# VealFang/PLI-SLAM

Hardware: AMD Instinct MI355X
Metric: stereo frames/sec (ORB+LSD extract+match), 752x480 EuRoC (higher is better)
Workload: dtype u8; 1 GPU; 1xMI355X: 752x480 stereo pairs, extract + stereo Hamming match (BASELINE configs[1] shape, batched); 752x480, 1200 ORB kp (8 levels x1.2) + LSD/LBD (<=100 lines); 256 stereo frames per GPU per step; frames_per_gpu=256, parallelism=frame-batch data parallel, 1 rank(s), gather of result tables to rank 0

## Files before the change

### pli_slam_amd/csrc/lsd_rect.hpp

```cpp
#pragma once
#include "kernels.hpp"
#include "device_prims.hpp"

namespace pli {

constexpr double RX_PI = 3.14159265358979323846;
constexpr double RX_DEG2RAD = RX_PI / 180;
constexpr double RX_3_2_PI = (3 * RX_PI) / 2;
constexpr double RX_2PI = 2 * RX_PI;

__device__ __forceinline__ double rx_angle_diff(double a, double b) {
  double diff = a - b;
  while (diff <= -RX_PI) diff += RX_2PI;
  while (diff > RX_PI) diff -= RX_2PI;
  return fabs(diff);
}

constexpr int RX_RECT_GROUP_MAX = 192;
constexpr int RX_RECT_CACHE = 4;

template <int LANES>
__device__ __forceinline__ void rx_rect_region(bool on, const RxRect& it, const DevParams& P, const float4* __restrict__ rec,
                                               const double* __restrict__ mg, const int* __restrict__ arena,
                                               float4* __restrict__ rgSeg, double (*st)[64], double (*wc)[64], int (*ec)[64], int rmask,
                                               const int2* __restrict__ hot = nullptr ,
                                               const float2* __restrict__ cold = nullptr ) {
  const int lane = threadIdx.x & 63, gl = lane & (LANES - 1), g0 = lane & ~(LANES - 1);
  const int W = P.LW;
  const double prec = P.prec;
  const int cnt = on ? it.cnt : 0;
  const int* lst = arena + it.off;
  const double reg_angle = (double)fast_atan2_deg(it.sumdy, it.sumdx) * RX_DEG2RAD;
  int cmax = cnt;
#pragma unroll
  for (int o = 32; o >= LANES; o >>= 1) cmax = max(cmax, __shfl_xor(cmax, o, 64));
  double acc = 0.0;
  for (int c0 = 0; c0 < cmax; c0 += LANES) {
    const int kk = c0 + gl;
    double v0 = 0.0, v1 = 0.0, v2 = 0.0;
    if (kk < cnt) {
      const int e = lst[kk];
      const int ex = e & 0xFFFF, ey = e >> 16;
      const double w = mg ? mg[ey * W + ex] : sqrt((double)__float_as_int(rec[ey * W + ex].w) / 4.0);
      v0 = (double)ex * w;
      v1 = (double)ey * w;
      v2 = w;
      if (c0 < RX_RECT_CACHE * LANES) { wc[c0 / LANES][lane] = w; ec[c0 / LANES][lane] = e; }
    }
    wave_lds_sync();
    st[0][lane] = v0; st[1][lane] = v1; st[2][lane] = v2;
    wave_lds_sync();
    if (gl < 3 && c0 < cnt) {
      const int mm = (min(LANES, cnt - c0) + 7) & ~7;
      for (int tt = 0; tt < mm; tt += 8) {
        double a[8];
#pragma unroll
        for (int u = 0; u < 8; ++u) a[u] = st[gl][g0 + tt + u];
#pragma unroll
        for (int u = 0; u < 8; ++u) acc += a[u];
      }
    }
  }
  const double cq = acc / __shfl(acc, g0 + 2, 64);
  const double x = __shfl(cq, g0, 64), y = __shfl(cq, g0 + 1, 64);
  acc = 0.0;
  for (int c0 = 0; c0 < cmax; c0 += LANES) {
    const int kk = c0 + gl;
    double v0 = 0.0, v1 = 0.0, v2 = 0.0;
    if (kk < cnt) {
      const bool cached = c0 < RX_RECT_CACHE * LANES;
      const int e = cached ? ec[c0 / LANES][lane] : lst[kk];
      const int ex = e & 0xFFFF, ey = e >> 16;
      const double w = cached ? wc[c0 / LANES][lane] : (mg ? mg[ey * W + ex] : sqrt((double)__float_as_int(rec[ey * W + ex].w) / 4.0));
      const double dx = (double)ex - x, dy = (double)ey - y;
      v0 = dy * dy * w;
      v1 = dx * dx * w;
      v2 = dx * dy * w;
    }
    wave_lds_sync();
    st[0][lane] = v0; st[1][lane] = v1; st[2][lane] = v2;
    wave_lds_sync();
    if (gl < 3 && c0 < cnt) {
      const int mm = (min(LANES, cnt - c0) + 7) & ~7;
      for (int tt = 0; tt < mm; tt += 8) {
        double a[8];
#pragma unroll
        for (int u = 0; u < 8; ++u) a[u] = st[gl][g0 + tt + u];
        if (gl < 2) {
#pragma unroll
          for (int u = 0; u < 8; ++u) acc += a[u];
        } else {
#pragma unroll
          for (int u = 0; u < 8; ++u) acc -= a[u];
        }
      }
    }
  }
  const double Ixx = __shfl(acc, g0, 64), Iyy = __shfl(acc, g0 + 1, 64), Ixy = __shfl(acc, g0 + 2, 64);
  const double lambda = 0.5 * (Ixx + Iyy - sqrt((Ixx - Iyy) * (Ixx - Iyy) + 4.0 * Ixy * Ixy));
  const bool wide = fabs(Ixx) > fabs(Iyy);
  double theta = (double)fast_atan2_deg(wide ? (float)(lambda - Ixx) : (float)Ixy, wide ? (float)Ixy : (float)(lambda - Iyy));
  theta *= RX_DEG2RAD;
  double adiff = rx_angle_diff(theta, reg_angle);
  {
    const bool need = on && it.approx != 0 && hot != nullptr && fabs(adiff - prec) < P.rectApproxBand;
    if (__builtin_amdgcn_ballot_w64(need)) {
      int cm = need ? cnt : 0;
#pragma unroll
      for (int o = 32; o >= LANES; o >>= 1) cm = max(cm, __shfl_xor(cm, o, 64));
      float sx = 0.f, sy = 0.f;
      for (int c0 = 0; c0 < cm; c0 += LANES) {
        const int kk = c0 + gl;
        float cy = 0.f, cz = 0.f;
        if (need && kk < cnt) {
          const int e = lst[kk];
          const int p = (e >> 16) * W + (e & 0xFFFF);
          if (kk == 0) {
            double sn, cs;
            sincos((double)__int_as_float(hot[p].x) * RX_DEG2RAD, &sn, &cs);
            cy = (float)cs; cz = (float)sn;
          } else if (cold) {
            const float2 cp = cold[p];
            cy = cp.x; cz = cp.y;
          } else {
            const float4 r = rec[p];
            cy = r.y; cz = r.z;
          }
        }
        for (int j = 0; j < LANES; ++j) {
          const float vy = __shfl(cy, g0 + j, 64), vz = __shfl(cz, g0 + j, 64);
          if (need && c0 + j < cnt) {
            sx = (c0 + j == 0) ? vy : __fadd_rn(sx, vy);
            sy = (c0 + j == 0) ? vz : __fadd_rn(sy, vz);
          }
        }
      }
      if (need) adiff = rx_angle_diff(theta, (double)fast_atan2_deg(sy, sx) * RX_DEG2RAD);
    }
  }
  if (adiff > prec) theta += RX_PI;
  double dxr, dyr;
  sincos(theta, &dyr, &dxr);
  double l_min = 0, l_max = 0;
  for (int kk = gl; kk < cnt; kk += LANES) {
    const int e = kk < RX_RECT_CACHE * LANES ? ec[kk / LANES][lane] : lst[kk];
    const double l = ((double)(e & 0xFFFF) - x) * dxr + ((double)(e >> 16) - y) * dyr;
    l_max = fmax(l_max, l);
    l_min = fmin(l_min, l);
  }
#pragma unroll
  for (int o = LANES / 2; o > 0; o >>= 1) {
    l_max = fmax(l_max, __shfl_xor(l_max, o, 64));
    l_min = fmin(l_min, __shfl_xor(l_min, o, 64));
  }
  double e = ((gl & 1) ? y : x) + ((gl & 2) ? l_max : l_min) * ((gl & 1) ? dyr : dxr);
  e += 0.5;
  const double scale = P.lsdScale;
  if (scale != 1) e /= scale;
  if (on && gl < 4) reinterpret_cast<float*>(&rgSeg[it.rank & rmask])[gl] = (float)e;
}


__device__ __forceinline__ void rx_rect_wave(const DevParams& P, const RxCtl& c, const float4* __restrict__ rec, const double* __restrict__ mg,
                                             const int* __restrict__ arena, const RxRect* __restrict__ rects, int rectCap,
                                             float4* __restrict__ rgSeg, int first, int stride, double (*st)[64], double (*wc)[64],
                                             int (*ec)[64], int rmask = -1, const int2* __restrict__ hot = nullptr,
                                             const float2* __restrict__ cold = nullptr) {
  const int nrect = min((int)(c.rectArena >> RX_ARENA_BITS), rectCap);
  const int lane = threadIdx.x & 63, g = lane >> 4;
  for (int w0 = first * 4; w0 < nrect; w0 += stride * 4) {
    RxRect it = {0, 0, 0, 1.f, 0.f, 0};
    const bool have = w0 + g < nrect;
    if (have) it = rects[w0 + g];
    const bool small = have && it.cnt <= RX_RECT_GROUP_MAX;
    if (__builtin_amdgcn_ballot_w64(small)) rx_rect_region<16>(small, it, P, rec, mg, arena, rgSeg, st, wc, ec, rmask, hot, cold);
    unsigned long long big = __builtin_amdgcn_ballot_w64(have && !small) & 0x0001000100010001ull;
    while (big) {
      const int gl0 = __ffsll((long long)big) - 1;
      big &= big - 1ull;
      RxRect bt;
      bt.rank = __shfl(it.rank, gl0, 64); bt.off = __shfl(it.off, gl0, 64); bt.cnt = __shfl(it.cnt, gl0, 64);
      bt.sumdx = __shfl(it.sumdx, gl0, 64); bt.sumdy = __shfl(it.sumdy, gl0, 64); bt.approx = __shfl(it.approx, gl0, 64);
      rx_rect_region<64>(true, bt, P, rec, mg, arena, rgSeg, st, wc, ec, rmask, hot, cold);
    }
  }
}

}
```

### pli_slam_amd/csrc/lsd_relax.hip

```cpp
#include "kernels.hpp"
#include "device_prims.hpp"
#include "lsd_rect.hpp"
#include <climits>
#include <type_traits>

namespace pli {

constexpr float RX_NOTDEF = -1024.f;
constexpr int RX_INF = LSD_ID_INF;

__device__ __forceinline__ int2 rx_load_own(const int2* p) {
  unsigned long long v = __hip_atomic_load(reinterpret_cast<const unsigned long long*>(p), __ATOMIC_RELAXED,
                                           __HIP_MEMORY_SCOPE_AGENT);
  return make_int2((int)(v & 0xFFFFFFFFull), (int)(v >> 32));
}

__device__ __forceinline__ int rx_lds_read(const int* p) {
  typedef __attribute__((address_space(3))) const volatile int lds_cvint;
  return *(lds_cvint*)p;
}


__device__ __forceinline__ int rx_block_append(bool flag, int* counter, int* lds) {
  const int tid = threadIdx.x, lane = tid & 63, wv = tid >> 6, nw = blockDim.x >> 6;
// ... 542 lines not shown
          cnt = 1; k = 0;
          bx0 = bx1 = sd.xy & 0xFFFF; by0 = by1 = sd.xy >> 16;
        } else {
          const RxHand& hd = hand[wi - nbig];
          r = hd.rank; cnt = hd.cnt; k = hd.k;
          sumdx = hd.sumdx; sumdy = hd.sumdy;
          reg_angle = (double)fast_atan2_deg(sumdy, sumdx) * RX_DEG2RAD;
          bx0 = hd.box0 & 0xFFFF; by0 = hd.box0 >> 16; bx1 = hd.box1 & 0xFFFF; by1 = hd.box1 >> 16;
          for (int i = gl; i < cnt; i += RX_GL) q[i] = hd.q[i];
        }
        r = U(r); cnt = U(cnt); k = U(k);
        bx0 = U(bx0); bx1 = U(bx1); by0 = U(by0); by1 = U(by1);
        sumdx = Uf(sumdx); sumdy = Uf(sumdy);
      }
    }
    if constexpr (RX_GL == 64) { active = U(active) != 0; exhausted = U(exhausted) != 0; }
    if (!__builtin_amdgcn_ballot_w64(active)) break;
    __builtin_amdgcn_fence(__ATOMIC_RELEASE, "wavefront");
    bool dead = false, accepted = false;
    int qi = 0, nb = 0;
    raced = raced || pendOld <= r;
    asm volatile("" ::"v"(pendOld) : "memory");
    pendOld = 0x7FFFFFFF;
    auto step = [&](auto spillTag) {
      constexpr bool SPILL = decltype(spillTag)::value;
      int myxy = -1;
      qi = -1;
      float4 rr = make_float4(RX_NOTDEF, 0.f, 0.f, 0.f);
      int2 oo = make_int2(0, 0);
      nb = active ? min(NP, cnt - k) : 0;
      if (pi < nb) {
        const int e = SPILL ? qget(k + pi) : rx_lds_read(&q[k + pi]);
        const int nx = (e & 0xFFFF) + ndx, ny = (e >> 16) + ndy;
        if (nx >= 0 && ny >= 0 && nx < W && ny < H) {
          qi = ny * W + nx;
          myxy = (ny << 16) | nx;
          rr = rec[qi];
          oo = rx_load_own(&own[qi]);
        }
      }
      const int prevv = ci ? oo.x : oo.y, curv = ci ? oo.y : oo.x;
      const bool cand = rr.x != RX_NOTDEF && !(prevv < r || curv <= r);
      const double ad = (double)rr.x * RX_DEG2RAD;
      unsigned long long rem = (__builtin_amdgcn_ballot_w64(cand) >> gbase) & GMASK;
      dead = false; accepted = false;
      while (__builtin_amdgcn_ballot_w64(rem != 0)) {
        double n_theta = fabs(reg_angle - ad);
        if (n_theta > RX_3_2_PI) {
          n_theta = fabs(n_theta - RX_2PI);
        }
        const unsigned long long m = ((__builtin_amdgcn_ballot_w64(cand && n_theta <= prec) >> gbase) & GMASK) & rem;
        if (!m) { rem = 0; continue; }
        const int j2 = __ffsll((long long)m) - 1;
        rem &= ~((2ull << j2) - 1ull);
        const float cj = bcast(rr.y, j2), sj = bcast(rr.z, j2);
        const int xyj = __float_as_int(bcast(__int_as_float(myxy), j2));
        const int qj = __float_as_int(bcast(__int_as_float(qi), j2));
        rem &= ~((__builtin_amdgcn_ballot_w64(qi == qj) >> gbase) & GMASK);
        const int ax = xyj & 0xFFFF, ay = xyj >> 16;
        accepted = accepted || gl == j2;
        if (!SPILL || cnt < RX_GQ) {
          q[cnt] = xyj;
        } else {
          const int o = cnt - RX_GQ;
          if (o % RX_BBLK == 0) {
            int nbk = 0;
            if (o / RX_BBLK >= RX_BMAXBLK) { dead = true; rem = 0; continue; }
            if (gl == 0) {
              const unsigned long long ra = atomicAdd(&c.rectArena, (unsigned long long)RX_BBLK) & ((1ull << RX_ARENA_BITS) - 1ull);
              nbk = ra + RX_BBLK > (unsigned long long)arenaCap ? -1 : (int)ra;
            }
            nbk = __shfl(nbk, gbase, 64);
            if (nbk < 0) { dead = true; rem = 0; continue; }
            gb[o / RX_BBLK] = nbk;
          }
          if (gl == 0) arena[gb[o / RX_BBLK] + o % RX_BBLK] = xyj;
          __threadfence_block();
        }
        ++cnt;
        bx0 = min(bx0, ax); bx1 = max(bx1, ax); by0 = min(by0, ay); by1 = max(by1, ay);
        sumdx = __fadd_rn(sumdx, cj);
        sumdy = __fadd_rn(sumdy, sj);
        reg_angle = (double)fast_atan2_deg(sumdy, sumdx) * RX_DEG2RAD;
      }
    };
    if (__builtin_amdgcn_ballot_w64(active && cnt + 8 * NP + 1 > RX_GQ)) step(std::true_type{});
    else step(std::false_type{});
    if (accepted) pendOld = __hip_atomic_fetch_min(ci ? &own[qi].y : &own[qi].x, r, __ATOMIC_RELAXED, __HIP_MEMORY_SCOPE_AGENT);
    if (active) {
      k += nb;
      if (dead) { c.overflow = 5; active = false; exhausted = true; }
      else if (k >= cnt) {
        active = false;
        if (raced || pendOld <= r) atomicAdd(&c.races, 1);
        raced = false; pendOld = 0x7FFFFFFF;
        if (gl == 0) {
          rgSize[r] = cnt;
          rgBox[r] = make_int2((by0 << 16) | bx0, (by1 << 16) | bx1);
        }
        if (cnt >= minReg) {
          int off = 0, slot = 0;
          if (gl == 0) {
            const unsigned long long ra = atomicAdd(&c.rectArena, (1ull << RX_ARENA_BITS) | (unsigned long long)cnt);
            const unsigned long long o64 = ra & ((1ull << RX_ARENA_BITS) - 1ull);
            off = o64 + cnt > (unsigned long long)arenaCap ? -1 : (int)o64;
            slot = (int)(ra >> RX_ARENA_BITS);
          }
          off = __shfl(off, gbase, 64); slot = __shfl(slot, gbase, 64);
          if (off < 0 || slot >= rectCap) c.overflow = off < 0 ? 3 : 4;
          else {
            for (int i = gl; i < cnt; i += RX_GL) arena[off + i] = qget(i);
            if (gl == 0) {
              RxRect& it = rects[slot];
              it.rank = r; it.off = off; it.cnt = cnt; it.sumdx = sumdx; it.sumdy = sumdy; it.approx = 0;
            }
          }
        }
      }
    }
  }
}

__global__ __launch_bounds__(64) void k_rx_grow_big(const DevParams* __restrict__ Pp, RxCtl* __restrict__ ctl,
                                                    const float4* __restrict__ recAll, int2* __restrict__ ownAll,
                                                    const RxSeed* __restrict__ bigAll, int bigCap,
                                                    const RxHand* __restrict__ handAll, int handCap,
                                                    int* __restrict__ rgSizeAll, int2* __restrict__ rgBoxAll,
                                                    int* __restrict__ arenaAll, int arenaCap,
                                                    RxRect* __restrict__ rectAll, int rectCap, int img0, int t) {
  rx_grow_groups<32, 512>(Pp, ctl, recAll, ownAll, bigAll, bigCap, handAll, handCap, rgSizeAll, rgBoxAll, arenaAll, arenaCap,
                          rectAll, rectCap, img0, t);
}

__global__ __launch_bounds__(64) void k_rx_grow_wave(const DevParams* __restrict__ Pp, RxCtl* __restrict__ ctl,
                                                     const float4* __restrict__ recAll, int2* __restrict__ ownAll,
                                                     const RxSeed* __restrict__ bigAll, int bigCap,
                                                     const RxHand* __restrict__ handAll, int handCap,
                                                     int* __restrict__ rgSizeAll, int2* __restrict__ rgBoxAll,
                                                     int* __restrict__ arenaAll, int arenaCap,
                                                     RxRect* __restrict__ rectAll, int rectCap, int img0, int t) {
  rx_grow_groups<64, 1024>(Pp, ctl, recAll, ownAll, bigAll, bigCap, handAll, handCap, rgSizeAll, rgBoxAll, arenaAll, arenaCap,
                           rectAll, rectCap, img0, t);
}

#endif

__global__ __launch_bounds__(64) void k_rx_rect(const DevParams* __restrict__ Pp, RxCtl* __restrict__ ctl,
                                                const float4* __restrict__ recAll, const int* __restrict__ arenaAll,
                                                int arenaCap, const RxRect* __restrict__ rectAll, int rectCap,
                                                float4* __restrict__ rgSegAll, int img0, const double* __restrict__ mgAll, int rmask,
                                                const int2* __restrict__ hotAll ,
                                                const float2* __restrict__ coldAll ) {
  __shared__ double st[3][64];
  __shared__ double wc[RX_RECT_CACHE][64];
  __shared__ int ec[RX_RECT_CACHE][64];
  const DevParams& P = *Pp;
  const int img = blockIdx.y + img0;
  const RxCtl& c = ctl[img];
  if (c.state == 2 || c.overflow) return;
  const int64_t npix = (int64_t)P.LW * P.LH;
  rx_rect_wave(P, c, recAll + img * npix, mgAll ? mgAll + img * npix : nullptr ,
               arenaAll + (int64_t)img * arenaCap, rectAll + (int64_t)img * rectCap, rectCap, rgSegAll + img * npix, blockIdx.x, gridDim.x, st, wc, ec, rmask,
               hotAll ? hotAll + img * npix : nullptr, coldAll ? coldAll + img * npix : nullptr);
}

constexpr int RX_CCHUNK = 2048;

__device__ __forceinline__ bool rx_emits(const int* order, const int2* own, int size, int i, int n, int minReg, const int2* box, int boxCut) {
  if (i >= n) return false;
  if (size < minReg || own[order[i]].x != i) return false;
  if (boxCut < 0) return true;
  const int2 b = box[i];
  return lsd_box_can_pass(b.x, b.y, boxCut);
}

__global__ __launch_bounds__(256) void k_rx_count(const RxCtl* __restrict__ ctl, const int* __restrict__ orderAll,
                                                  const int* __restrict__ nDefined, const int2* __restrict__ ownAll,
                                                  const int* __restrict__ rgSizeAll, int* __restrict__ chunkCntAll,
                                                  int nChunks, int64_t npix, int minReg, int img0, const int2* __restrict__ rgBoxAll,
                                                  int boxCut) {
  __shared__ int wsum[4];
  const int img = blockIdx.y + img0;
  if (ctl[img].state != 2 || ctl[img].overflow) return;
  const int n = nDefined[img];
  const int tid = threadIdx.x;
  int cntv = 0;
  int sz[RX_CCHUNK / 256];
#pragma unroll
  for (int j = 0; j < RX_CCHUNK / 256; ++j) sz[j] = rgSizeAll[img * npix + min((int)blockIdx.x * RX_CCHUNK + j * 256 + tid, max(n - 1, 0))];
#pragma unroll
  for (int j = 0; j < RX_CCHUNK / 256; ++j)
    cntv += rx_emits(orderAll + img * npix, ownAll + img * npix, sz[j], blockIdx.x * RX_CCHUNK + j * 256 + tid, n, minReg,
                     rgBoxAll + img * npix, boxCut) ? 1 : 0;
  cntv = wave_sum_i32(cntv);
  if ((tid & 63) == 0) wsum[tid >> 6] = cntv;
  __syncthreads();
  if (tid == 0) chunkCntAll[(int64_t)img * nChunks + blockIdx.x] = wsum[0] + wsum[1] + wsum[2] + wsum[3];
}

__global__ __launch_bounds__(256) void k_rx_emit(const RxCtl* __restrict__ ctl, const int* __restrict__ orderAll,
                                                 const int* __restrict__ nDefined, const int2* __restrict__ ownAll,
                                                 const int* __restrict__ rgSizeAll, const float4* __restrict__ rgSegAll,
                                                 const int* __restrict__ chunkCntAll, int nChunks, int64_t npix,
                                                 int minReg, float* __restrict__ segAll, int* __restrict__ nSeg,
                                                 int maxSeg, int img0, const int2* __restrict__ rgBoxAll, int boxCut) {
  __shared__ int wsum[4];
  __shared__ int sbase;
  const int img = blockIdx.y + img0;
  if (ctl[img].state != 2 || ctl[img].overflow) return;
  const int n = nDefined[img];
  const int tid = threadIdx.x, lane = tid & 63, wv = tid >> 6;
  const int* cc = chunkCntAll + (int64_t)img * nChunks;
  int part = 0;
  for (int j = tid; j < (int)blockIdx.x; j += 256) part += cc[j];
  part = wave_sum_i32(part);
  if (lane == 0) wsum[wv] = part;
  __syncthreads();
  if (tid == 0) sbase = wsum[0] + wsum[1] + wsum[2] + wsum[3];
  __syncthreads();
  int base = sbase;
  float* seg = segAll + (int64_t)img * maxSeg * 4;
  int sz[RX_CCHUNK / 256];
#pragma unroll
  for (int j = 0; j < RX_CCHUNK / 256; ++j) sz[j] = rgSizeAll[img * npix + min((int)blockIdx.x * RX_CCHUNK + j * 256 + tid, max(n - 1, 0))];
#pragma unroll
  for (int j = 0; j < RX_CCHUNK / 256; ++j) {
    const int i = blockIdx.x * RX_CCHUNK + j * 256 + tid;
    const bool e = rx_emits(orderAll + img * npix, ownAll + img * npix, sz[j], i, n, minReg, rgBoxAll + img * npix, boxCut);
    const unsigned long long bal = __builtin_amdgcn_ballot_w64(e);
    __syncthreads();
    if (lane == 0) wsum[wv] = __popcll(bal);
    __syncthreads();
    int pos = base + __popcll(bal & ((1ull << lane) - 1ull));
    for (int w2 = 0; w2 < wv; ++w2) pos += wsum[w2];
    if (e && pos < maxSeg) {
      const float4 v = rgSegAll[img * npix + i];
      seg[4 * pos + 0] = v.x; seg[4 * pos + 1] = v.y; seg[4 * pos + 2] = v.z; seg[4 * pos + 3] = v.w;
    }
    base += wsum[0] + wsum[1] + wsum[2] + wsum[3];
  }
  if ((int)blockIdx.x == nChunks - 1 && tid == 0) nSeg[img] = min(base, maxSeg);
}

}
```

### pli_slam_amd/csrc/lsd_tile.hip

```cpp
#include "kernels.hpp"
#include "device_prims.hpp"
#include "lsd_rect.hpp"
#include <climits>
#include <type_traits>

namespace pli {

constexpr float TX_NOTDEF = -1024.f;
constexpr int TX_INF = LSD_ID_INF;
constexpr double TX_PI = 3.14159265358979323846;
constexpr double TX_DEG2RAD = TX_PI / 180;
constexpr double TX_3_2_PI = (3 * TX_PI) / 2;
constexpr double TX_2PI = 2 * TX_PI;
#if !defined(PLI_DEV) && (defined(TX_CLAIM_SCOPE) || defined(TX_GROUP) || defined(TX_OWN_LOAD) || defined(TX_DIAG_PAD) || defined(TX_DIAG_NOWAIT) || defined(TX_DIAG_HOT_NOFOLD))
#error "diagnostic builds of lsd_tile.hip need -DPLI_DEV"
#endif
#ifndef TX_CLAIM_SCOPE
#define TX_CLAIM_SCOPE __HIP_MEMORY_SCOPE_AGENT
#endif
#ifndef TX_GROUP
#define TX_GROUP 8
#endif
static_assert(TX_GROUP == 0 || TX_GROUP == 2 || TX_GROUP == 4 || TX_GROUP == 8, "a group member is an octet of lanes");
constexpr int TX_GQ = 768;
// ... 1776 lines not shown
}
#ifdef PLI_DEV
__global__ __launch_bounds__(64) __attribute__((amdgpu_waves_per_eu(8, 8))) void k_tx_grow_spec(TxRound A, int t) {
  __shared__ int q[TX_GQ_SPEC];
  __shared__ int gb[TX_BMAXBLK];
  __shared__ int park[8 * 64];
  tx_grow_tile<false, true, TX_GQ_SPEC>(A, blockIdx.y + A.img0, blockIdx.x, t, q, gb, park);
}
#endif
__global__ __launch_bounds__(64) __attribute__((amdgpu_waves_per_eu(8, 8))) void k_tx_grow_sparse(TxRound A, int t) {
  __shared__ int q[TX_GQ];
  __shared__ int gb[TX_BMAXBLK];
  __shared__ int park[TX_PARK];
  tx_grow_tile<true>(A, blockIdx.y + A.img0, blockIdx.x, t, q, gb, park);
}
__global__ __launch_bounds__(64) __attribute__((amdgpu_waves_per_eu(8, 8))) void k_tx_grow_sparse_h(TxRound A, int t) {
  __shared__ int q[TX_GQ];
  __shared__ int gb[TX_BMAXBLK + 4];
  __shared__ int park[TX_PARK];
  tx_grow_tile<true, false, TX_GQ, 0, true>(A, blockIdx.y + A.img0, blockIdx.x, t, q, gb, park);
}

__global__ __launch_bounds__(256) void k_tx_rec_from_hot(const RxCtl* __restrict__ ctl, const int2* __restrict__ hotAll,
                                                         const float2* __restrict__ coldAll, float4* __restrict__ recAll, int64_t npix, int img0) {
  const int img = blockIdx.y + img0;
  if (ctl[img].state == 2 && ctl[img].overflow == 0) return;
  for (int64_t p = (int64_t)blockIdx.x * 256 + threadIdx.x; p < npix; p += (int64_t)gridDim.x * 256) {
    const float2 cp = coldAll[img * npix + p];
    recAll[img * npix + p] = make_float4(__int_as_float(hotAll[img * npix + p].x), cp.x == TX_NOTDEF ? 0.f : cp.x, cp.y, 0.f);
  }
}


__global__ __launch_bounds__(256) void k_tx_collect(RxCtl* __restrict__ ctl, const int* __restrict__ idPlaneAll, const int2* __restrict__ ownAll,
                                                    const int* __restrict__ rgSizeAll, int64_t npix, int minReg, int* __restrict__ candAll,
                                                    int* __restrict__ candCnt, int img0, int emitCap, const int2* __restrict__ rgBoxAll,
                                                    int boxCut) {
  constexpr int CAP = 1024;
  __shared__ int s_n, s_base;
  __shared__ int s_buf[CAP];
  const int img = blockIdx.y + img0;
  RxCtl& c = ctl[img];
  if (c.state != 2 || c.overflow) return;
  const int64_t base = (int64_t)img * npix;
  const int tid = threadIdx.x, lane = tid & 63;
  int* cand = candAll + (int64_t)img * TX_EMIT_CAP;
  if (tid == 0) s_n = 0;
  __syncthreads();
  const int* rgSize = rgSizeAll + base;
  const bool vec = (npix & 3) == 0 && ((uintptr_t)rgSize & 15) == 0;
  for (int64_t p1 = (int64_t)blockIdx.x * 4096; p1 < npix; p1 += (int64_t)gridDim.x * 4096) {
    int sz[16];
#pragma unroll
    for (int u = 0; u < 4; ++u) {
      const int64_t p = p1 + u * 1024 + tid * 4;
      int4 v = make_int4(0, 0, 0, 0);
      if (vec && p + 3 < npix) v = *reinterpret_cast<const int4*>(rgSize + p);
      else {
        if (p < npix) v.x = rgSize[p];
        if (p + 1 < npix) v.y = rgSize[p + 1];
        if (p + 2 < npix) v.z = rgSize[p + 2];
        if (p + 3 < npix) v.w = rgSize[p + 3];
      }
      sz[4 * u] = v.x; sz[4 * u + 1] = v.y; sz[4 * u + 2] = v.z; sz[4 * u + 3] = v.w;
    }
    unsigned hits = 0u;
#pragma unroll
    for (int j = 0; j < 16; ++j) hits |= (sz[j] >= minReg ? 1u : 0u) << j;
    while (hits) {
      const int j = __ffs(hits) - 1;
      hits &= hits - 1u;
      const int64_t p = p1 + (j >> 2) * 1024 + tid * 4 + (j & 3);
      const int id = idPlaneAll[base + p];
      const int2 box = boxCut >= 0 ? rgBoxAll[base + p] : make_int2(0, 0);
      if (id == TX_INF || ownAll[base + p].x != id || !lsd_box_can_pass(box.x, box.y, boxCut)) continue;
      const int at = atomicAdd(&s_n, 1);
      if (at < CAP) s_buf[at] = id;
      else {
        const int g = atomicAdd(&candCnt[img], 1);
        if (g < emitCap) cand[g] = id;
        else c.overflow = 6;
      }
    }
  }
  __syncthreads();
  const int n = min(s_n, CAP);
  if (tid == 0 && n) s_base = atomicAdd(&candCnt[img], n);
  __syncthreads();
  for (int i = tid; i < n; i += 256) {
    if (s_base + i < emitCap) cand[s_base + i] = s_buf[i];
    else c.overflow = 6;
  }
}

template <int KPT>
__device__ __forceinline__ void tx_emit_sort(unsigned* ks, const int* __restrict__ cand, int n, int tid) {
  unsigned key[KPT];
#pragma unroll
  for (int u = 0; u < KPT; ++u) key[u] = tid * KPT + u < n ? (unsigned)cand[tid * KPT + u] : 0xFFFFFFFFu;
  tx_bitonic_regs<KPT, 1024>(key, ks, tid);
  __syncthreads();
#pragma unroll
  for (int u = 0; u < KPT; ++u) ks[tid * KPT + u] = key[u];
  __syncthreads();
}

__global__ __launch_bounds__(1024) void k_tx_emit_sorted(const RxCtl* __restrict__ ctl, const int* __restrict__ candAll, const int* __restrict__ candCnt,
                                                         const float4* __restrict__ rgSegAll, int64_t npix, int rmask, float* __restrict__ segAll,
                                                         int* __restrict__ nSeg, int maxSeg, int img0, int emitCap) {
  extern __shared__ unsigned ks[];
  const int img = blockIdx.x + img0;
  if (ctl[img].state != 2 || ctl[img].overflow) return;
  const int n = min(candCnt[img], emitCap), tid = threadIdx.x;
  const int* cand = candAll + (int64_t)img * TX_EMIT_CAP;
  if (n <= 1024) tx_emit_sort<1>(ks, cand, n, tid);
  else if (n <= 2048) tx_emit_sort<2>(ks, cand, n, tid);
  else if (n <= 4096) tx_emit_sort<4>(ks, cand, n, tid);
  else if (n <= 8192) tx_emit_sort<8>(ks, cand, n, tid);
  else tx_emit_sort<16>(ks, cand, n, tid);
  float* seg = segAll + (int64_t)img * maxSeg * 4;
  for (int i = tid; i < min(n, maxSeg); i += 1024) {
    const float4 v = rgSegAll[img * npix + (int)(ks[i] & (unsigned)rmask)];
    seg[4 * i + 0] = v.x; seg[4 * i + 1] = v.y; seg[4 * i + 2] = v.z; seg[4 * i + 3] = v.w;
  }
  if (tid == 0) nSeg[img] = min(n, maxSeg);
}

__device__ __forceinline__ bool tx_grid_barrier(unsigned* bar, unsigned target) {
  __shared__ int s_ok;
  asm volatile("s_waitcnt vmcnt(0) lgkmcnt(0)" ::: "memory");
  __syncthreads();
  if (threadIdx.x == 0) {
    __builtin_amdgcn_fence(__ATOMIC_RELEASE, "agent");
    __hip_atomic_fetch_add(&bar[0], 1u, __ATOMIC_RELAXED, __HIP_MEMORY_SCOPE_AGENT);
    int ok = 1;
    unsigned spins = 0;
    while (__hip_atomic_load(&bar[0], __ATOMIC_RELAXED, __HIP_MEMORY_SCOPE_AGENT) < target) {
      __builtin_amdgcn_s_sleep(4);
      if ((++spins & 63u) == 0u &&
          (__hip_atomic_load(&bar[32], __ATOMIC_RELAXED, __HIP_MEMORY_SCOPE_AGENT) != 0u || spins > (1u << 21))) {
        __hip_atomic_store(&bar[32], 1u, __ATOMIC_RELAXED, __HIP_MEMORY_SCOPE_AGENT);
        ok = 0;
        break;
      }
    }
    __builtin_amdgcn_fence(__ATOMIC_ACQUIRE, "agent");
    s_ok = ok;
  }
  __syncthreads();
  asm volatile("s_dcache_inv" ::: "memory");
  return s_ok != 0;
}

__global__ __launch_bounds__(256) void k_tx_tail(TxTailArgs T) {
  __shared__ int qs[4][TX_GQ];
  __shared__ int gbs[4][TX_BMAXBLK + 4];
  __shared__ int parks[4][TX_PARK];
  __shared__ double sts[4][3][64];
  __shared__ double wcs[4][RX_RECT_CACHE][64];
  __shared__ int ecs[4][RX_RECT_CACHE][64];
  __shared__ int s_live, s_n;
  __shared__ int s_list[256];
  if (T.forceAbort) {
    if (threadIdx.x == 0) __hip_atomic_store(&T.bar[32], 1u, __ATOMIC_RELAXED, __HIP_MEMORY_SCOPE_AGENT);
    return;
  }
  const TxRound& A = T.R;
  const DevParams& P = *A.Pp;
  const int W = A.W, H = A.H;
  const int64_t npix = (int64_t)W * H;
  const int tid = threadIdx.x, wv = tid >> 6;
  const int G = gridDim.x;
  const int nbx = (W + 31) / 32, nbyA = (A.TH + 7) / 8, nbyB = (H + 31) / 32, ntile = A.ntx * A.nty, ncell = A.TW * A.TH;
  const int64_t nA = (int64_t)nbx * nbyA * A.nimg, nB = (int64_t)nbx * nbyB * A.nimg, nC = (int64_t)ntile * A.nimg;
  const int nwaves = G * 4, gw = blockIdx.x * 4 + wv;
  auto relaxing = [&](int il) -> bool {
    const RxCtl& c = A.ctl[A.img0 + il];
    return c.state != 2 && c.overflow == 0;
  };
  unsigned epoch = 0;
  for (int t = T.t0; t <= T.maxRounds; ++t) {
    for (int il = blockIdx.x * 256 + tid; il < A.nimg; il += G * 256) {
      RxCtl& c = A.ctl[A.img0 + il];
      if (c.state != 2) { c.nSmall = 0; c.nBig = 0; c.nHand = 0; c.nextBig = 0; c.rectArena = 0ull; }
    }
    for (int64_t base = blockIdx.x; base < nA; base += (int64_t)G * 256) {
      if (tid == 0) s_n = 0;
      __syncthreads();
      const int64_t v = base + (int64_t)tid * G;
      if (v < nA) {
        const int il = (int)(v / (nbx * nbyA)), rem = (int)(v - (int64_t)il * (nbx * nbyA));
        const int bx = rem % nbx, by = rem / nbx;
        bool act = false;
        if (relaxing(il)) {
          const int* tt = A.tileTouch + (int64_t)(A.img0 + il) * ncell;
          for (int cy = by * 8; cy < min(by * 8 + 8, A.TH); ++cy)
            for (int cx = bx * 4; cx < min(bx * 4 + 4, A.TW); ++cx) act = act || tt[cy * A.TW + cx] == t - 1;
        }
        if (act) s_list[atomicAdd(&s_n, 1)] = (int)((v - base) / G);
      }
      __syncthreads();
      const int n = s_n;
      for (int i = 0; i < n; ++i) {
        const int64_t va = base + (int64_t)s_list[i] * G;
        const int il = (int)(va / (nbx * nbyA)), rem = (int)(va - (int64_t)il * (nbx * nbyA));
        tx_diffmark_block(A, t, rem % nbx, rem / nbx, A.img0 + il);
        __syncthreads();
      }
    }
    if (!tx_grid_barrier(T.bar, ++epoch * G)) return;
    for (int il = blockIdx.x * 256 + tid; il < A.nimg; il += G * 256) {
      RxCtl& c = A.ctl[A.img0 + il];
      if (c.state == 2) continue;
      if (((t & 1) ? c.changedOdd : c.changed) == 0) { c.state = 2; c.rounds = t; }
      else if (t & 1) c.changed = 0;
      else c.changedOdd = 0;
    }
    for (int64_t base = blockIdx.x; base < nB; base += (int64_t)G * 256) {
      if (tid == 0) s_n = 0;
      __syncthreads();
      const int64_t v = base + (int64_t)tid * G;
      if (v < nB) {
        const int il = (int)(v / (nbx * nbyB)), rem = (int)(v - (int64_t)il * (nbx * nbyB));
        const int bx = rem % nbx, by = rem / nbx;
        bool act = false;
        if (relaxing(il)) {
          const int* ta = A.tileAct + (int64_t)(A.img0 + il) * ncell;
          for (int cy = by * 4; cy < min(by * 4 + 4, A.TH); ++cy)
            for (int cx = bx * 4; cx < min(bx * 4 + 4, A.TW); ++cx) act = act || ta[cy * A.TW + cx] == t;
        }
        if (act) s_list[atomicAdd(&s_n, 1)] = (int)((v - base) / G);
      }
      __syncthreads();
      const int n = s_n;
      for (int i = 0; i < n; ++i) {
        const int64_t va = base + (int64_t)s_list[i] * G;
        const int il = (int)(va / (nbx * nbyB)), rem = (int)(va - (int64_t)il * (nbx * nbyB));
        tx_prep_block(A, t, rem % nbx, rem / nbx, A.img0 + il, 0);
        __syncthreads();
      }
    }
    if (!tx_grid_barrier(T.bar, ++epoch * G)) return;
    if (tid == 0) s_live = 0;
    __syncthreads();
    int live = 0;
    for (int i = tid; i < A.nimg; i += 256) live += relaxing(i) ? 1 : 0;
    if (live) atomicAdd(&s_live, live);
    __syncthreads();
    if (s_live == 0) return;
    for (int64_t base = blockIdx.x; base < nC; base += (int64_t)G * 256) {
      if (tid == 0) s_n = 0;
      __syncthreads();
      const int64_t v = base + (int64_t)tid * G;
      if (v < nC && A.DL.cnt[(int64_t)A.img0 * ntile + v] > 0 && relaxing((int)(v / ntile))) s_list[atomicAdd(&s_n, 1)] = (int)((v - base) / G);
      __syncthreads();
      const int n = s_n;
      for (int i = wv; i < n; i += 4) {
        const int64_t va = base + (int64_t)s_list[i] * G;
        const int il = (int)(va / ntile);
        const int tile = (int)(va - (int64_t)il * ntile);
        if (A.hot) tx_grow_tile<true, false, TX_GQ, 0, true>(A, A.img0 + il, tile, t, qs[wv], gbs[wv], parks[wv]);
        else tx_grow_tile<true>(A, A.img0 + il, tile, t, qs[wv], gbs[wv], parks[wv]);
      }
      __syncthreads();
    }
    if (!tx_grid_barrier(T.bar, ++epoch * G)) return;
    for (int64_t v = (int64_t)blockIdx.x * 256 + tid; v < nC; v += (int64_t)G * 256) A.DL.cnt[(int64_t)A.img0 * ntile + v] = 0;
    {
      const int per = max(1, nwaves / A.nimg);
      for (int il = gw / per; il < A.nimg; il += max(1, nwaves / per)) {
        const int img = A.img0 + il;
        const RxCtl& c = A.ctl[img];
        if (c.state == 2 || c.overflow) continue;
        rx_rect_wave(P, c, A.rec + img * npix, A.mg ? A.mg + img * npix : nullptr, A.arena + (int64_t)img * A.arenaCap,
                     A.rects + (int64_t)img * A.rectCap, A.rectCap, A.rgSeg + img * npix, gw % per, per, sts[wv], wcs[wv], ecs[wv], A.DL.rmask,
                     A.hot ? A.hot + img * npix : nullptr, A.cold ? A.cold + img * npix : nullptr);
      }
    }
    if (!tx_grid_barrier(T.bar, ++epoch * G)) return;
  }
}

}
```

Before: 6977 stereo frames/s.

## Prefetch rect point lists into registers and software-pipeline rect descriptor loads

Adds a PRE variant of the LSD rectangle fitting that batches the gather of point indices and gradient weights into register arrays with all loads issued up front, instead of one dependent load per 16/64-lane chunk, and drops the LDS cache of weights and indices. The rect descriptor for the next iteration is also loaded one iteration ahead. The standalone relax kernel uses the new path; the fused tail kernel keeps the old one via a constexpr flag. It raises register pressure and, for 64-lane regions, reloads indices and weights for blocks beyond the first on each pass.

```diff
diff --git a/pli_slam_amd/csrc/lsd_rect.hpp b/pli_slam_amd/csrc/lsd_rect.hpp
--- a/pli_slam_amd/csrc/lsd_rect.hpp
+++ b/pli_slam_amd/csrc/lsd_rect.hpp
@@ -1,4 +1,5 @@
 #pragma once
+#include <type_traits>
 #include "kernels.hpp"
 #include "device_prims.hpp"
 
@@ -18,8 +19,9 @@
 
 constexpr int RX_RECT_GROUP_MAX = 192;
 constexpr int RX_RECT_CACHE = 4;
-
-template <int LANES>
+constexpr int RX_RECT_WAVE_BLOCK = 4;
+
+template <int LANES, bool PRE>
 __device__ __forceinline__ void rx_rect_region(bool on, const RxRect& it, const DevParams& P, const float4* __restrict__ rec,
                                                const double* __restrict__ mg, const int* __restrict__ arena,
                                                float4* __restrict__ rgSeg, double (*st)[64], double (*wc)[64], int (*ec)[64], int rmask,
@@ -34,19 +36,8 @@
   int cmax = cnt;
 #pragma unroll
   for (int o = 32; o >= LANES; o >>= 1) cmax = max(cmax, __shfl_xor(cmax, o, 64));
-  double acc = 0.0;
-  for (int c0 = 0; c0 < cmax; c0 += LANES) {
-    const int kk = c0 + gl;
-    double v0 = 0.0, v1 = 0.0, v2 = 0.0;
-    if (kk < cnt) {
-      const int e = lst[kk];
-      const int ex = e & 0xFFFF, ey = e >> 16;
-      const double w = mg ? mg[ey * W + ex] : sqrt((double)__float_as_int(rec[ey * W + ex].w) / 4.0);
-      v0 = (double)ex * w;
-      v1 = (double)ey * w;
-      v2 = w;
-      if (c0 < RX_RECT_CACHE * LANES) { wc[c0 / LANES][lane] = w; ec[c0 / LANES][lane] = e; }
-    }
+
+  auto ordered = [&](auto second, const int c0, const double v0, const double v1, const double v2, double& acc) {
     wave_lds_sync();
     st[0][lane] = v0; st[1][lane] = v1; st[2][lane] = v2;
     wave_lds_sync();
@@ -56,44 +47,140 @@
         double a[8];
 #pragma unroll
         for (int u = 0; u < 8; ++u) a[u] = st[gl][g0 + tt + u];
-#pragma unroll
-        for (int u = 0; u < 8; ++u) acc += a[u];
-      }
+        if (!decltype(second)::value || gl < 2) {
+#pragma unroll
+          for (int u = 0; u < 8; ++u) acc += a[u];
+        } else {
+#pragma unroll
+          for (int u = 0; u < 8; ++u) acc -= a[u];
+        }
+      }
+    }
+  };
+  const auto weight_of = [&](const int ex, const int ey) -> double {
+    return mg ? mg[ey * W + ex] : sqrt((double)__float_as_int(rec[ey * W + ex].w) / 4.0);
+  };
+
+  constexpr int NB = LANES == 16 ? RX_RECT_GROUP_MAX / 16 : RX_RECT_WAVE_BLOCK;
+  constexpr int BLOCK = NB * LANES;
+  static_assert(LANES == 64 || BLOCK == RX_RECT_GROUP_MAX, "a 16-lane group holds its whole list");
+  auto fetch = [&](auto nt, const int b0, int (&e)[NB], double (&w)[NB], const bool weights) {
+    constexpr int N = decltype(nt)::value;
+    const int last = max(cnt - 1, 0);
+#pragma unroll
+    for (int c = 0; c < N; ++c) {
+      int kk = min(b0 + c * LANES + gl, last);
+      asm("" : "+v"(kk));
+      e[c] = lst[kk];
+    }
+    __builtin_amdgcn_sched_barrier(0);
+    if (!weights) return;
+    if (mg) {
+#pragma unroll
+      for (int c = 0; c < N; ++c) {
+        int p = cnt > 0 ? (e[c] >> 16) * W + (e[c] & 0xFFFF) : 0;
+        asm("" : "+v"(p));
+        w[c] = mg[p];
+      }
+      __builtin_amdgcn_sched_barrier(0);
+    } else {
+      float r[N];
+#pragma unroll
+      for (int c = 0; c < N; ++c) {
+        int p = cnt > 0 ? (e[c] >> 16) * W + (e[c] & 0xFFFF) : 0;
+        asm("" : "+v"(p));
+        r[c] = rec[p].w;
+      }
+      __builtin_amdgcn_sched_barrier(0);
+#pragma unroll
+      for (int c = 0; c < N; ++c) w[c] = sqrt((double)__float_as_int(r[c]) / 4.0);
+    }
+  };
+  auto fetch_block = [&](const int b0, int (&e)[NB], double (&w)[NB], const bool weights) {
+    if (cmax - b0 > BLOCK / 2) fetch(std::integral_constant<int, NB>{}, b0, e, w, weights);
+    else fetch(std::integral_constant<int, NB / 2>{}, b0, e, w, weights);
+  };
+  auto sums1_block = [&](const int b0, const int (&e)[NB], const double (&w)[NB], double& acc) {
+#pragma unroll
+    for (int c = 0; c < NB; ++c) {
+      const int c0 = b0 + c * LANES;
+      if (c0 < cmax) {
+        const bool in = c0 + gl < cnt;
+        const int ex = e[c] & 0xFFFF, ey = e[c] >> 16;
+        ordered(std::false_type{}, c0, in ? (double)ex * w[c] : 0.0, in ? (double)ey * w[c] : 0.0, in ? w[c] : 0.0, acc);
+      }
+    }
+  };
+  auto sums2_block = [&](const int b0, const int (&e)[NB], const double (&w)[NB], const double x, const double y, double& acc) {
+#pragma unroll
+    for (int c = 0; c < NB; ++c) {
+      const int c0 = b0 + c * LANES;
+      if (c0 < cmax) {
+        const bool in = c0 + gl < cnt;
+        const double dx = (double)(e[c] & 0xFFFF) - x, dy = (double)(e[c] >> 16) - y;
+        ordered(std::true_type{}, c0, in ? dy * dy * w[c] : 0.0, in ? dx * dx * w[c] : 0.0, in ? dx * dy * w[c] : 0.0, acc);
+      }
+    }
+  };
+  int ek[NB] = {};
+  double wk[NB] = {};
+
+  double acc = 0.0;
+  if constexpr (PRE) {
+    fetch_block(0, ek, wk, true);
+    sums1_block(0, ek, wk, acc);
+    if constexpr (LANES == 64) {
+      for (int b0 = BLOCK; b0 < cmax; b0 += BLOCK) {
+        int eb[NB] = {};
+        double wb[NB] = {};
+        fetch_block(b0, eb, wb, true);
+        sums1_block(b0, eb, wb, acc);
+      }
+    }
+  } else {
+    for (int c0 = 0; c0 < cmax; c0 += LANES) {
+      const int kk = c0 + gl;
+      double v0 = 0.0, v1 = 0.0, v2 = 0.0;
+      if (kk < cnt) {
+        const int e = lst[kk];
+        const int ex = e & 0xFFFF, ey = e >> 16;
+        const double w = weight_of(ex, ey);
+        v0 = (double)ex * w;
+        v1 = (double)ey * w;
+        v2 = w;
+        if (c0 < RX_RECT_CACHE * LANES) { wc[c0 / LANES][lane] = w; ec[c0 / LANES][lane] = e; }
+      }
+      ordered(std::false_type{}, c0, v0, v1, v2, acc);
     }
   }
   const double cq = acc / __shfl(acc, g0 + 2, 64);
   const double x = __shfl(cq, g0, 64), y = __shfl(cq, g0 + 1, 64);
   acc = 0.0;
-  for (int c0 = 0; c0 < cmax; c0 += LANES) {
-    const int kk = c0 + gl;
-    double v0 = 0.0, v1 = 0.0, v2 = 0.0;
-    if (kk < cnt) {
-      const bool cached = c0 < RX_RECT_CACHE * LANES;
-      const int e = cached ? ec[c0 / LANES][lane] : lst[kk];
-      const int ex = e & 0xFFFF, ey = e >> 16;
-      const double w = cached ? wc[c0 / LANES][lane] : (mg ? mg[ey * W + ex] : sqrt((double)__float_as_int(rec[ey * W + ex].w) / 4.0));
-      const double dx = (double)ex - x, dy = (double)ey - y;
-      v0 = dy * dy * w;
-      v1 = dx * dx * w;
-      v2 = dx * dy * w;
-    }
-    wave_lds_sync();
-    st[0][lane] = v0; st[1][lane] = v1; st[2][lane] = v2;
-    wave_lds_sync();
-    if (gl < 3 && c0 < cnt) {
-      const int mm = (min(LANES, cnt - c0) + 7) & ~7;
-      for (int tt = 0; tt < mm; tt += 8) {
-        double a[8];
-#pragma unroll
-        for (int u = 0; u < 8; ++u) a[u] = st[gl][g0 + tt + u];
-        if (gl < 2) {
-#pragma unroll
-          for (int u = 0; u < 8; ++u) acc += a[u];
-        } else {
-#pragma unroll
-          for (int u = 0; u < 8; ++u) acc -= a[u];
-        }
-      }
+  if constexpr (PRE) {
+    sums2_block(0, ek, wk, x, y, acc);
+    if constexpr (LANES == 64) {
+      for (int b0 = BLOCK; b0 < cmax; b0 += BLOCK) {
+        int eb[NB] = {};
+        double wb[NB] = {};
+        fetch_block(b0, eb, wb, true);
+        sums2_block(b0, eb, wb, x, y, acc);
+      }
+    }
+  } else {
+    for (int c0 = 0; c0 < cmax; c0 += LANES) {
+      const int kk = c0 + gl;
+      double v0 = 0.0, v1 = 0.0, v2 = 0.0;
+      if (kk < cnt) {
+        const bool cached = c0 < RX_RECT_CACHE * LANES;
+        const int e = cached ? ec[c0 / LANES][lane] : lst[kk];
+        const int ex = e & 0xFFFF, ey = e >> 16;
+        const double w = cached ? wc[c0 / LANES][lane] : weight_of(ex, ey);
+        const double dx = (double)ex - x, dy = (double)ey - y;
+        v0 = dy * dy * w;
+        v1 = dx * dx * w;
+        v2 = dx * dy * w;
+      }
+      ordered(std::true_type{}, c0, v0, v1, v2, acc);
     }
   }
   const double Ixx = __shfl(acc, g0, 64), Iyy = __shfl(acc, g0 + 1, 64), Ixy = __shfl(acc, g0 + 2, 64);
@@ -142,11 +229,32 @@
   double dxr, dyr;
   sincos(theta, &dyr, &dxr);
   double l_min = 0, l_max = 0;
-  for (int kk = gl; kk < cnt; kk += LANES) {
-    const int e = kk < RX_RECT_CACHE * LANES ? ec[kk / LANES][lane] : lst[kk];
-    const double l = ((double)(e & 0xFFFF) - x) * dxr + ((double)(e >> 16) - y) * dyr;
-    l_max = fmax(l_max, l);
-    l_min = fmin(l_min, l);
+  if constexpr (PRE) {
+    auto ends_block = [&](const int b0, const int (&e)[NB]) {
+#pragma unroll
+      for (int c = 0; c < NB; ++c)
+        if (b0 + c * LANES + gl < cnt) {
+          const double l = ((double)(e[c] & 0xFFFF) - x) * dxr + ((double)(e[c] >> 16) - y) * dyr;
+          l_max = fmax(l_max, l);
+          l_min = fmin(l_min, l);
+        }
+    };
+    ends_block(0, ek);
+    if constexpr (LANES == 64) {
+      for (int b0 = BLOCK; b0 < cmax; b0 += BLOCK) {
+        int eb[NB] = {};
+        double wb[NB] = {};
+        fetch_block(b0, eb, wb, false);
+        ends_block(b0, eb);
+      }
+    }
+  } else {
+    for (int kk = gl; kk < cnt; kk += LANES) {
+      const int e = kk < RX_RECT_CACHE * LANES ? ec[kk / LANES][lane] : lst[kk];
+      const double l = ((double)(e & 0xFFFF) - x) * dxr + ((double)(e >> 16) - y) * dyr;
+      l_max = fmax(l_max, l);
+      l_min = fmin(l_min, l);
+    }
   }
 #pragma unroll
   for (int o = LANES / 2; o > 0; o >>= 1) {
@@ -161,6 +269,7 @@
 }
 
 
+template <bool PRE>
 __device__ __forceinline__ void rx_rect_wave(const DevParams& P, const RxCtl& c, const float4* __restrict__ rec, const double* __restrict__ mg,
                                              const int* __restrict__ arena, const RxRect* __restrict__ rects, int rectCap,
                                              float4* __restrict__ rgSeg, int first, int stride, double (*st)[64], double (*wc)[64],
@@ -168,12 +277,24 @@
                                              const float2* __restrict__ cold = nullptr) {
   const int nrect = min((int)(c.rectArena >> RX_ARENA_BITS), rectCap);
   const int lane = threadIdx.x & 63, g = lane >> 4;
+  if (first * 4 >= nrect) return;
+  const RxRect none = {0, 0, 0, 1.f, 0.f, 0};
+  RxRect nx = none;
+  if constexpr (PRE) nx = rects[min(first * 4 + g, nrect - 1)];
   for (int w0 = first * 4; w0 < nrect; w0 += stride * 4) {
-    RxRect it = {0, 0, 0, 1.f, 0.f, 0};
+    RxRect it = none;
     const bool have = w0 + g < nrect;
-    if (have) it = rects[w0 + g];
+    if constexpr (PRE) {
+      it.rank = have ? nx.rank : none.rank; it.off = have ? nx.off : none.off; it.cnt = have ? nx.cnt : none.cnt;
+      it.sumdx = have ? nx.sumdx : none.sumdx; it.sumdy = have ? nx.sumdy : none.sumdy; it.approx = have ? nx.approx : none.approx;
+      int at = min(w0 + stride * 4 + g, nrect - 1);
+      asm("" : "+v"(at));
+      nx = rects[at];
+    } else {
+      if (have) it = rects[w0 + g];
+    }
     const bool small = have && it.cnt <= RX_RECT_GROUP_MAX;
-    if (__builtin_amdgcn_ballot_w64(small)) rx_rect_region<16>(small, it, P, rec, mg, arena, rgSeg, st, wc, ec, rmask, hot, cold);
+    if (__builtin_amdgcn_ballot_w64(small)) rx_rect_region<16, PRE>(small, it, P, rec, mg, arena, rgSeg, st, wc, ec, rmask, hot, cold);
     unsigned long long big = __builtin_amdgcn_ballot_w64(have && !small) & 0x0001000100010001ull;
     while (big) {
       const int gl0 = __ffsll((long long)big) - 1;
@@ -181,7 +302,7 @@
       RxRect bt;
       bt.rank = __shfl(it.rank, gl0, 64); bt.off = __shfl(it.off, gl0, 64); bt.cnt = __shfl(it.cnt, gl0, 64);
       bt.sumdx = __shfl(it.sumdx, gl0, 64); bt.sumdy = __shfl(it.sumdy, gl0, 64); bt.approx = __shfl(it.approx, gl0, 64);
-      rx_rect_region<64>(true, bt, P, rec, mg, arena, rgSeg, st, wc, ec, rmask, hot, cold);
+      rx_rect_region<64, PRE>(true, bt, P, rec, mg, arena, rgSeg, st, wc, ec, rmask, hot, cold);
     }
   }
 }
diff --git a/pli_slam_amd/csrc/lsd_relax.hip b/pli_slam_amd/csrc/lsd_relax.hip
--- a/pli_slam_amd/csrc/lsd_relax.hip
+++ b/pli_slam_amd/csrc/lsd_relax.hip
@@ -718,15 +718,13 @@
                                                 const int2* __restrict__ hotAll ,
                                                 const float2* __restrict__ coldAll ) {
   __shared__ double st[3][64];
-  __shared__ double wc[RX_RECT_CACHE][64];
-  __shared__ int ec[RX_RECT_CACHE][64];
   const DevParams& P = *Pp;
   const int img = blockIdx.y + img0;
   const RxCtl& c = ctl[img];
   if (c.state == 2 || c.overflow) return;
   const int64_t npix = (int64_t)P.LW * P.LH;
-  rx_rect_wave(P, c, recAll + img * npix, mgAll ? mgAll + img * npix : nullptr ,
-               arenaAll + (int64_t)img * arenaCap, rectAll + (int64_t)img * rectCap, rectCap, rgSegAll + img * npix, blockIdx.x, gridDim.x, st, wc, ec, rmask,
+  rx_rect_wave<true>(P, c, recAll + img * npix, mgAll ? mgAll + img * npix : nullptr ,
+               arenaAll + (int64_t)img * arenaCap, rectAll + (int64_t)img * rectCap, rectCap, rgSegAll + img * npix, blockIdx.x, gridDim.x, st, nullptr, nullptr, rmask,
                hotAll ? hotAll + img * npix : nullptr, coldAll ? coldAll + img * npix : nullptr);
 }
 
diff --git a/pli_slam_amd/csrc/lsd_tile.hip b/pli_slam_amd/csrc/lsd_tile.hip
--- a/pli_slam_amd/csrc/lsd_tile.hip
+++ b/pli_slam_amd/csrc/lsd_tile.hip
@@ -1952,6 +1952,7 @@
   return s_ok != 0;
 }
 
+constexpr bool TX_TAIL_RECT_PRE = false;
 __global__ __launch_bounds__(256) void k_tx_tail(TxTailArgs T) {
   __shared__ int qs[4][TX_GQ];
   __shared__ int gbs[4][TX_BMAXBLK + 4];
@@ -2072,7 +2073,7 @@
         const int img = A.img0 + il;
         const RxCtl& c = A.ctl[img];
         if (c.state == 2 || c.overflow) continue;
-        rx_rect_wave(P, c, A.rec + img * npix, A.mg ? A.mg + img * npix : nullptr, A.arena + (int64_t)img * A.arenaCap,
+        rx_rect_wave<TX_TAIL_RECT_PRE>(P, c, A.rec + img * npix, A.mg ? A.mg + img * npix : nullptr, A.arena + (int64_t)img * A.arenaCap,
                      A.rects + (int64_t)img * A.rectCap, A.rectCap, A.rgSeg + img * npix, gw % per, per, sts[wv], wcs[wv], ecs[wv], A.DL.rmask,
                      A.hot ? A.hot + img * npix : nullptr, A.cold ? A.cold + img * npix : nullptr);
       }
```

Measured after the change: 7091 stereo frames/s (median of 6 runs). 1.02x the previous value.
